# russellgeum/Digging-into-Self-Supervised-Monocular-Depth-Estimation

Hardware: AMD Instinct MI355X
Metric: images/sec training, KITTI 192x640 batch 12/GPU (higher is better)
Workload: dtype f32; 1 GPU; configs[1]: kitti_eigen_zhou-shaped 192x640, batch 12/GPU, ResNet18 depth + separate ResNet18 pose, frame_ids [0,-1,1], 4 scales, automask, Adam, fp32; global_batch=12, parallelism=dp1

## Files before the change

### digging-into-self-supervised-monocular-depth-estimation_amd/csrc/norm_nhwc.hip

```cpp
#include "nhwc_common.hpp"

namespace mdx {
namespace nhwc {

constexpr int STATS_FWD_BLOCKS = 256;
constexpr int STATS_BWD_BLOCKS_F32 = 256, STATS_BWD_BLOCKS_BF16 = 384;
constexpr int STATS_MAX_BLOCKS = 384;
constexpr int APPLY_MAX_BLOCKS = 4096;
constexpr int STATS_ITERS = 8, APPLY_ITERS = 4;
static inline int stats_bwd_blocks(int dtype) { return dtype == MDX_F32 ? STATS_BWD_BLOCKS_F32 : STATS_BWD_BLOCKS_BF16; }

template <typename T>
__global__ __launch_bounds__(NB) void bn_nhwc_fwd_stats_kernel(const T *__restrict__ x, int M, int C, int CVB, int PL, int RB,
                                                               float *__restrict__ part)
{
    constexpr int N = VecN<T>::N;
    __shared__ float lds[2 * NB * N];
    const Pos p = position<N>(M, C, CVB, PL, RB);
    float a[N], q[N];
#pragma unroll
    for (int j = 0; j < N; ++j) a[j] = q[j] = 0.f;
    if (p.active) {
        const T *px = x + (size_t)p.g * M * C + (size_t)p.cv * N;
        auto acc = [&](const Vec<T, N> &v) {
#pragma unroll
            for (int j = 0; j < N; ++j) {
                const float f = to_float(v.v[j]);
                a[j] += f;
                q[j] = __builtin_fmaf(f, f, q[j]);
            }
        };
        int r = p.r0 + p.pl;
        for (; r + 3 * PL < p.r1; r += 4 * PL) {
            const Vec<T, N> v0 = load_vec<T, N>(px + (size_t)r * C), v1 = load_vec<T, N>(px + (size_t)(r + PL) * C);
            const Vec<T, N> v2 = load_vec<T, N>(px + (size_t)(r + 2 * PL) * C), v3 = load_vec<T, N>(px + (size_t)(r + 3 * PL) * C);
            acc(v0); acc(v1); acc(v2); acc(v3);
        }
        for (; r < p.r1; r += PL) acc(load_vec<T, N>(px + (size_t)r * C));
    }
    block_partials<N>(a, q, lds, CVB, PL, C, part + ((size_t)p.g * gridDim.x + blockIdx.x) * 2 * C);
}

constexpr int FC = 16, FS = 64, FU = STATS_MAX_BLOCKS / FS;
__device__ __forceinline__ void channel_totals(const float *__restrict__ part_g, int nblk, int C, int c, double (*lds)[FS / 4][FC],
                                               double &ta, double &tq)
{
    const int cl = threadIdx.x % FC, sl = threadIdx.x / FC;
    float va[FU], vq[FU];
#pragma unroll
    for (int i = 0; i < FU; ++i) {
        const int b = sl + i * FS;
        const bool ok = c < C && b < nblk;
        va[i] = ok ? part_g[(size_t)b * 2 * C + c] : 0.f;
        vq[i] = ok ? part_g[(size_t)b * 2 * C + C + c] : 0.f;
    }
    double a = 0.0, q = 0.0;
#pragma unroll
    for (int i = 0; i < FU; ++i) {
        a += (double)va[i];
        q += (double)vq[i];
    }
    a += __shfl_down(a, 32, 64);
    q += __shfl_down(q, 32, 64);
    a += __shfl_down(a, 16, 64);
    q += __shfl_down(q, 16, 64);
    if ((threadIdx.x & 63) < FC) {
        lds[0][threadIdx.x >> 6][cl] = a;
        lds[1][threadIdx.x >> 6][cl] = q;
    }
    __syncthreads();
    ta = tq = 0.0;
    if (threadIdx.x < FC)
#pragma unroll
        for (int s = 0; s < FS / 4; ++s) {
            ta += lds[0][s][cl];
            tq += lds[1][s][cl];
        }
    __syncthreads();
}

__global__ __launch_bounds__(FC *FS) void bn_nhwc_fwd_finalize_kernel(const float *__restrict__ part, int nblk, int C, int G, double M,
                                                                       float eps, float momentum, float *__restrict__ save_mean,
                                                                       float *__restrict__ save_invstd, float *__restrict__ run_mean,
                                                                       float *__restrict__ run_var)
{
    __shared__ double lds[2][FS / 4][FC];
    const int c = blockIdx.x * FC + threadIdx.x % FC;
    const bool writer = threadIdx.x < FC && c < C;
    float rm = 0.f, rv = 0.f;
    if (writer && run_mean) { rm = run_mean[c]; rv = run_var[c]; }
    for (int g = 0; g < G; ++g) {
        double a, q;
        channel_totals(part + (size_t)g * nblk * 2 * C, nblk, C, c, lds, a, q);
        if (writer) {
            const double m = a / M;
            double var = q / M - m * m;
            var = var > 0.0 ? var : 0.0;
            const float mean = (float)m;
            save_mean[(size_t)g * C + c] = mean;
            save_invstd[(size_t)g * C + c] = (float)(1.0 / sqrt(var + (double)eps));
            const double unbiased = M > 1.0 ? var * (M / (M - 1.0)) : var;
            rm = (1.0f - momentum) * rm + momentum * mean;
            rv = (1.0f - momentum) * rv + momentum * (float)unbiased;
        }
    }
    if (writer && run_mean) { run_mean[c] = rm; run_var[c] = rv; }
}

__global__ __launch_bounds__(FC *FS) void bn_nhwc_bwd_finalize_kernel(const float *__restrict__ part, int nblk, int C, int G, double M,
                                                                       float *__restrict__ totals, float *__restrict__ dgamma,
                                                                       float *__restrict__ dbeta)
{
    __shared__ double lds[2][FS / 4][FC];
    const int c = blockIdx.x * FC + threadIdx.x % FC;
    const bool writer = threadIdx.x < FC && c < C;
    float sa = 0.f, sq = 0.f;
    for (int g = 0; g < G; ++g) {
        double a, q;
        channel_totals(part + (size_t)g * nblk * 2 * C, nblk, C, c, lds, a, q);
        if (writer) {
            totals[((size_t)g * 2 + 0) * C + c] = (float)((double)(float)a / M);
            totals[((size_t)g * 2 + 1) * C + c] = (float)((double)(float)q / M);
            sa += (float)a;
            sq += (float)q;
        }
    }
    if (writer) { dbeta[c] = sa; dgamma[c] = sq; }
}

template <typename T>
__global__ __launch_bounds__(NB) void bn_nhwc_fwd_apply_kernel(const T *__restrict__ x, const T *__restrict__ res,
                                                               const float *__restrict__ gamma, const float *__restrict__ beta,
                                                               const float *__restrict__ save_mean,
                                                               const float *__restrict__ save_invstd, int M, int C, int CVB, int PL,
                                                               int RB, int relu, T *__restrict__ y)
{
    constexpr int N = VecN<T>::N;
    const Pos p = position<N>(M, C, CVB, PL, RB);
    if (!p.active) return;
    float scale[N], shift[N];
#pragma unroll
    for (int j = 0; j < N; ++j) {
        const int c = p.cv * N + j;
        scale[j] = gamma[c] * save_invstd[(size_t)p.g * C + c];
        shift[j] = beta[c] - save_mean[(size_t)p.g * C + c] * scale[j];
    }
    const size_t base = (size_t)p.g * M * C + (size_t)p.cv * N;
    const T *px = x + base;
    const T *pr = res ? res + base : nullptr;
    T *py = y + base;
    auto apply = [&](const Vec<T, N> &v, const Vec<T, N> &rv, size_t off) {
        Vec<T, N> w;
#pragma unroll
        for (int j = 0; j < N; ++j) {
            float f = __builtin_fmaf(to_float(v.v[j]), scale[j], shift[j]);
            if (pr) f += to_float(rv.v[j]);
            w.v[j] = from_float<T>((relu && f < 0.f) ? 0.f : f);
        }
        store_vec<T, N>(py + off, w);
    };
    int r = p.r0 + p.pl;
    for (; r + 3 * PL < p.r1; r += 4 * PL) {
        const size_t o0 = (size_t)r * C, o1 = (size_t)(r + PL) * C, o2 = (size_t)(r + 2 * PL) * C, o3 = (size_t)(r + 3 * PL) * C;
        const Vec<T, N> v0 = load_vec<T, N>(px + o0), v1 = load_vec<T, N>(px + o1), v2 = load_vec<T, N>(px + o2), v3 = load_vec<T, N>(px + o3);
        Vec<T, N> r0 = {}, r1 = {}, r2 = {}, r3 = {};
        if (pr) { r0 = load_vec<T, N>(pr + o0); r1 = load_vec<T, N>(pr + o1); r2 = load_vec<T, N>(pr + o2); r3 = load_vec<T, N>(pr + o3); }
        apply(v0, r0, o0); apply(v1, r1, o1); apply(v2, r2, o2); apply(v3, r3, o3);
    }
    for (; r < p.r1; r += PL) {
        const size_t o = (size_t)r * C;
        Vec<T, N> rv = {};
        if (pr) rv = load_vec<T, N>(pr + o);
        apply(load_vec<T, N>(px + o), rv, o);
    }
}

template <typename T, bool MASKX>
__global__ __launch_bounds__(NB) void bn_nhwc_bwd_stats_kernel(const T *__restrict__ dy, const T *__restrict__ dy2,
                                                               const T *__restrict__ y, const T *__restrict__ x,
                                                               const float *__restrict__ gamma, const float *__restrict__ beta,
                                                               const float *__restrict__ save_mean,
                                                               const float *__restrict__ save_invstd, int M, int C, int CVB, int PL,
                                                               int RB, int relu, float *__restrict__ part)
{
    constexpr int N = VecN<T>::N;
    __shared__ float lds[2 * NB * N];
    const Pos p = position<N>(M, C, CVB, PL, RB);
    float a[N], q[N];
#pragma unroll
    for (int j = 0; j < N; ++j) a[j] = q[j] = 0.f;
    if (p.active) {
        float mean[N], invstd[N], scale[N], shift[N];
#pragma unroll
        for (int j = 0; j < N; ++j) {
            mean[j] = save_mean[(size_t)p.g * C + p.cv * N + j];
            invstd[j] = save_invstd[(size_t)p.g * C + p.cv * N + j];
            scale[j] = shift[j] = 0.f;
            if (MASKX) {
                scale[j] = gamma[p.cv * N + j] * invstd[j];
                shift[j] = beta[p.cv * N + j] - mean[j] * scale[j];
            }
        }
        const size_t base = (size_t)p.g * M * C + (size_t)p.cv * N;
        const T *pd = dy + base, *pd2 = dy2 ? dy2 + base : nullptr, *py = MASKX ? nullptr : y + base, *px = x + base;
        auto acc = [&](const Vec<T, N> &vd, const Vec<T, N> &vd2, const Vec<T, N> &vy, const Vec<T, N> &vx) {
#pragma unroll
            for (int j = 0; j < N; ++j) {
                float d = to_float(vd.v[j]);
                if (pd2) d += to_float(vd2.v[j]);
                const float yv = !MASKX ? to_float(vy.v[j]) : to_float(from_float<T>(__builtin_fmaf(to_float(vx.v[j]), scale[j], shift[j])));
                const float dz = (relu && !(yv > 0.f)) ? 0.f : d;
                a[j] += dz;
                q[j] = __builtin_fmaf(dz, (to_float(vx.v[j]) - mean[j]) * invstd[j], q[j]);
            }
        };
        int r = p.r0 + p.pl;
        for (; r + PL < p.r1; r += 2 * PL) {
            const size_t o0 = (size_t)r * C, o1 = (size_t)(r + PL) * C;
            const Vec<T, N> d0 = load_vec<T, N>(pd + o0), d1 = load_vec<T, N>(pd + o1);
            Vec<T, N> y0 = {}, y1 = {};
            if (!MASKX) { y0 = load_vec<T, N>(py + o0); y1 = load_vec<T, N>(py + o1); }
            const Vec<T, N> x0 = load_vec<T, N>(px + o0), x1 = load_vec<T, N>(px + o1);
            Vec<T, N> e0 = {}, e1 = {};
            if (pd2) { e0 = load_vec<T, N>(pd2 + o0); e1 = load_vec<T, N>(pd2 + o1); }
            acc(d0, e0, y0, x0);
            acc(d1, e1, y1, x1);
        }
        for (; r < p.r1; r += PL) {
            const size_t o = (size_t)r * C;
            Vec<T, N> e = {}, yv = {};
            if (pd2) e = load_vec<T, N>(pd2 + o);
            if (!MASKX) yv = load_vec<T, N>(py + o);
            acc(load_vec<T, N>(pd + o), e, yv, load_vec<T, N>(px + o));
        }
    }
    block_partials<N>(a, q, lds, CVB, PL, C, part + ((size_t)p.g * gridDim.x + blockIdx.x) * 2 * C);
}

template <typename T, bool MASKX>
__global__ __launch_bounds__(NB) void bn_nhwc_bwd_apply_kernel(const T *__restrict__ dy, const T *__restrict__ dy2,
                                                               const T *__restrict__ y, const T *__restrict__ x,
                                                               const float *__restrict__ gamma, const float *__restrict__ beta,
                                                               const float *__restrict__ save_mean,
                                                               const float *__restrict__ save_invstd,
                                                               const float *__restrict__ totals, int M, int C, int CVB, int PL,
                                                               int RB, int relu, T *__restrict__ dx, T *__restrict__ dres)
{
    constexpr int N = VecN<T>::N;
    const Pos p = position<N>(M, C, CVB, PL, RB);
    if (!p.active) return;
    float mean[N], invstd[N], k0[N], mdz[N], mdzx[N], shift[N];
#pragma unroll
    for (int j = 0; j < N; ++j) {
        const int c = p.cv * N + j;
        mean[j] = save_mean[(size_t)p.g * C + c];
        invstd[j] = save_invstd[(size_t)p.g * C + c];
        k0[j] = gamma[c] * invstd[j];
        shift[j] = MASKX ? beta[c] - mean[j] * k0[j] : 0.f;
        mdz[j] = totals[((size_t)p.g * 2 + 0) * C + c];
        mdzx[j] = totals[((size_t)p.g * 2 + 1) * C + c];
    }
    const size_t base = (size_t)p.g * M * C + (size_t)p.cv * N;
    const T *pd = dy + base, *pd2 = dy2 ? dy2 + base : nullptr, *py = MASKX ? nullptr : y + base, *px = x + base;
    T *ox = dx + base;
    T *orr = dres ? dres + base : nullptr;
    auto apply = [&](const Vec<T, N> &vd, const Vec<T, N> &vd2, const Vec<T, N> &vy, const Vec<T, N> &vx, size_t off) {
        Vec<T, N> wx, wr;
#pragma unroll
        for (int j = 0; j < N; ++j) {
            float d = to_float(vd.v[j]);
            if (pd2) d += to_float(vd2.v[j]);
            const float yv = !MASKX ? to_float(vy.v[j]) : to_float(from_float<T>(__builtin_fmaf(to_float(vx.v[j]), k0[j], shift[j])));
            const float dz = (relu && !(yv > 0.f)) ? 0.f : d;
            const float xh = (to_float(vx.v[j]) - mean[j]) * invstd[j];
            wx.v[j] = from_float<T>(k0[j] * (dz - mdz[j] - xh * mdzx[j]));
            wr.v[j] = from_float<T>(dz);
        }
        store_vec<T, N>(ox + off, wx);
        if (orr) store_vec<T, N>(orr + off, wr);
    };
    int r = p.r0 + p.pl;
    for (; r + PL < p.r1; r += 2 * PL) {
        const size_t o0 = (size_t)r * C, o1 = (size_t)(r + PL) * C;
        const Vec<T, N> d0 = load_vec<T, N>(pd + o0), d1 = load_vec<T, N>(pd + o1);
        Vec<T, N> y0 = {}, y1 = {};
        if (!MASKX) { y0 = load_vec<T, N>(py + o0); y1 = load_vec<T, N>(py + o1); }
        const Vec<T, N> x0 = load_vec<T, N>(px + o0), x1 = load_vec<T, N>(px + o1);
        Vec<T, N> e0 = {}, e1 = {};
        if (pd2) { e0 = load_vec<T, N>(pd2 + o0); e1 = load_vec<T, N>(pd2 + o1); }
        apply(d0, e0, y0, x0, o0);
        apply(d1, e1, y1, x1, o1);
    }
    for (; r < p.r1; r += PL) {
        const size_t o = (size_t)r * C;
        Vec<T, N> e = {}, yv = {};
        if (pd2) e = load_vec<T, N>(pd2 + o);
        if (!MASKX) yv = load_vec<T, N>(py + o);
        apply(load_vec<T, N>(pd + o), e, yv, load_vec<T, N>(px + o), o);
    }
}

}
}

using namespace mdx;
using namespace mdx::nhwc;

MDX_EXPORT size_t mdx_bn_nhwc_workspace_bytes(int B, int C, int H, int W, int groups, int dtype)
{
    if (B <= 0 || C <= 0 || H <= 0 || W <= 0 || groups <= 0 || !dtype_ok(dtype)) return 0;
    const Rows g = make_rows((long long)B * H * W, C, vec_elems(dtype), STATS_MAX_BLOCKS, STATS_ITERS);
    return ((size_t)groups * g.nblk * 2 * C + (size_t)groups * 2 * C) * sizeof(float);
}

static int nhwc_args_ok(int B, int C, int H, int W, int groups, int dtype)
{
    if (groups <= 0 || groups > 65535) return MDX_ERR_BAD_SHAPE;
    return nhwc_map_ok(B, C, H, W, dtype);
}

MDX_EXPORT int mdx_bn_act_nhwc_fwd(const void *x, const void *res, const float *gamma, const float *beta, float *run_mean,
                                   float *run_var, void *y, float *save_mean, float *save_invstd, int B, int C, int H, int W,
                                   int groups, float eps, float momentum, int relu, int dtype, void *workspace,
                                   size_t workspace_bytes, void *stream)
{
    if (!x || !gamma || !beta || !y || !save_mean || !save_invstd || !workspace) return MDX_ERR_NULL_POINTER;
    if ((run_mean == nullptr) != (run_var == nullptr)) return MDX_ERR_NULL_POINTER;
    const int bad = nhwc_args_ok(B, C, H, W, groups, dtype);
    if (bad) return bad;
    if (!aligned(x, 16) || !aligned(y, 16) || (res && !aligned(res, 16))) return MDX_ERR_MISALIGNED;
    if (workspace_bytes < mdx_bn_nhwc_workspace_bytes(B, C, H, W, groups, dtype)) return MDX_ERR_WORKSPACE;
    const int M = B * H * W, N = vec_elems(dtype);
    const Rows gs = make_rows(M, C, N, STATS_FWD_BLOCKS, STATS_ITERS), ga = make_rows(M, C, N, APPLY_MAX_BLOCKS, APPLY_ITERS);
    float *part = (float *)workspace;
    hipStream_t st = (hipStream_t)stream;
    const dim3 grid_s(gs.nblk, gs.t.ny, groups), grid_a(ga.nblk, ga.t.ny, groups), block(NB);
    dispatch_dtype(dtype, [&](auto t) {
        using T = typename decltype(t)::type;
        hipLaunchKernelGGL((bn_nhwc_fwd_stats_kernel<T>), grid_s, block, 0, st, (const T *)x, M, C, gs.t.CVB, gs.t.PL, gs.RB, part);
    });
    hipLaunchKernelGGL(bn_nhwc_fwd_finalize_kernel, dim3((C + FC - 1) / FC), dim3(FC * FS), 0, st, part, gs.nblk, C, groups, (double)M,
                       eps, momentum, save_mean, save_invstd, run_mean, run_var);
    dispatch_dtype(dtype, [&](auto t) {
        using T = typename decltype(t)::type;
        hipLaunchKernelGGL((bn_nhwc_fwd_apply_kernel<T>), grid_a, block, 0, st, (const T *)x, (const T *)res, gamma, beta, save_mean,
                           save_invstd, M, C, ga.t.CVB, ga.t.PL, ga.RB, relu, (T *)y);
    });
    return check_launch();
}

MDX_EXPORT int mdx_bn_act_nhwc_bwd(const void *dy, const void *dy2, const void *y, const void *x, const float *gamma,
                                   const float *beta, const float *save_mean, const float *save_invstd, void *dx, void *dres, float *dgamma,
                                   float *dbeta, int B, int C, int H, int W, int groups, int relu, int dtype, void *workspace,
                                   size_t workspace_bytes, void *stream)
{
    if (!dy || !x || !gamma || !save_mean || !save_invstd || !dx || !dgamma || !dbeta || !workspace)
        return MDX_ERR_NULL_POINTER;
    if (!y && (!relu || !beta || dres)) return MDX_ERR_NULL_POINTER;
    const int bad = nhwc_args_ok(B, C, H, W, groups, dtype);
    if (bad) return bad;
    if (!aligned(dy, 16) || (y && !aligned(y, 16)) || !aligned(x, 16) || !aligned(dx, 16) || (dy2 && !aligned(dy2, 16)) ||
        (dres && !aligned(dres, 16)))
        return MDX_ERR_MISALIGNED;
    if (workspace_bytes < mdx_bn_nhwc_workspace_bytes(B, C, H, W, groups, dtype)) return MDX_ERR_WORKSPACE;
    const int M = B * H * W, N = vec_elems(dtype);
    const Rows gs = make_rows(M, C, N, stats_bwd_blocks(dtype), STATS_ITERS), ga = make_rows(M, C, N, APPLY_MAX_BLOCKS, APPLY_ITERS);
    float *part = (float *)workspace;
    float *totals = part + (size_t)groups * gs.nblk * 2 * C;
    hipStream_t st = (hipStream_t)stream;
    const dim3 grid_s(gs.nblk, gs.t.ny, groups), grid_a(ga.nblk, ga.t.ny, groups), block(NB);
    const bool maskx = !y;
    dispatch_dtype_flag(dtype, maskx, [&](auto t, auto mx) {
        using T = typename decltype(t)::type;
        hipLaunchKernelGGL((bn_nhwc_bwd_stats_kernel<T, decltype(mx)::value>), grid_s, block, 0, st, (const T *)dy, (const T *)dy2,
                           (const T *)y, (const T *)x, gamma, beta, save_mean, save_invstd, M, C, gs.t.CVB, gs.t.PL, gs.RB, relu, part);
    });
    hipLaunchKernelGGL(bn_nhwc_bwd_finalize_kernel, dim3((C + FC - 1) / FC), dim3(FC * FS), 0, st, part, gs.nblk, C, groups, (double)M, totals,
                       dgamma, dbeta);
    dispatch_dtype_flag(dtype, maskx, [&](auto t, auto mx) {
        using T = typename decltype(t)::type;
        hipLaunchKernelGGL((bn_nhwc_bwd_apply_kernel<T, decltype(mx)::value>), grid_a, block, 0, st, (const T *)dy, (const T *)dy2,
                           (const T *)y, (const T *)x, gamma, beta, save_mean, save_invstd, totals, M, C, ga.t.CVB, ga.t.PL, ga.RB, relu,
                           (T *)dx, (T *)dres);
    });
    return check_launch();
}
```

### digging-into-self-supervised-monocular-depth-estimation_amd/csrc/pose_head_nhwc.hip

```cpp
#include "nhwc_common.hpp"

namespace mdx {
namespace nhwc {

constexpr int BA_BLOCKS = 256, BA_ITERS = 4;

template <typename T>
__global__ __launch_bounds__(NB) void bias_act_nhwc_fwd_kernel(const T *__restrict__ x, const float *__restrict__ bias, int M, int C,
                                                               int CVB, int PL, int RB, int relu, T *__restrict__ y)
{
    constexpr int N = VecN<T>::N;
    const Pos p = position<N>(M, C, CVB, PL, RB);
    if (!p.active) return;
    float b[N];
#pragma unroll
    for (int j = 0; j < N; ++j) b[j] = bias[p.cv * N + j];
    const T *px = x + (size_t)p.cv * N;
    T *py = y + (size_t)p.cv * N;
    for (int r = p.r0 + p.pl; r < p.r1; r += PL) {
        const Vec<T, N> v = load_vec<T, N>(px + (size_t)r * C);
        Vec<T, N> w;
#pragma unroll
        for (int j = 0; j < N; ++j) {
            const float f = to_float(v.v[j]) + b[j];
            w.v[j] = from_float<T>((relu && f < 0.f) ? 0.f : f);
        }
        store_vec<T, N>(py + (size_t)r * C, w);
    }
}

template <typename T>
__global__ __launch_bounds__(NB) void bias_act_nhwc_bwd_kernel(const T *__restrict__ dy, const T *__restrict__ y, int M, int C, int CVB,
                                                               int PL, int RB, int relu, T *__restrict__ dx, float *__restrict__ part)
{
    constexpr int N = VecN<T>::N;
    __shared__ float lds[NB * N];
    const Pos p = position<N>(M, C, CVB, PL, RB);
    float a[N];
#pragma unroll
    for (int j = 0; j < N; ++j) a[j] = 0.f;
    if (p.active) {
        const T *__restrict__ pd = dy + (size_t)p.cv * N, *__restrict__ py = y + (size_t)p.cv * N;
        T *__restrict__ ox = dx + (size_t)p.cv * N;
        auto one = [&](const Vec<T, N> &d, const Vec<T, N> &v, size_t off) {
            Vec<T, N> w;
#pragma unroll
            for (int j = 0; j < N; ++j) {
                const float dz = (relu && !(to_float(v.v[j]) > 0.f)) ? 0.f : to_float(d.v[j]);
                a[j] += dz;
                w.v[j] = from_float<T>(dz);
            }
            store_vec<T, N>(ox + off, w);
        };
        int r = p.r0 + p.pl;
        for (; r + 3 * PL < p.r1; r += 4 * PL) {
            const size_t o0 = (size_t)r * C, o1 = (size_t)(r + PL) * C, o2 = (size_t)(r + 2 * PL) * C, o3 = (size_t)(r + 3 * PL) * C;
            const Vec<T, N> d0 = load_vec<T, N>(pd + o0), d1 = load_vec<T, N>(pd + o1), d2 = load_vec<T, N>(pd + o2), d3 = load_vec<T, N>(pd + o3);
            const Vec<T, N> v0 = load_vec<T, N>(py + o0), v1 = load_vec<T, N>(py + o1), v2 = load_vec<T, N>(py + o2), v3 = load_vec<T, N>(py + o3);
            one(d0, v0, o0); one(d1, v1, o1); one(d2, v2, o2); one(d3, v3, o3);
        }
        for (; r < p.r1; r += PL) one(load_vec<T, N>(pd + (size_t)r * C), load_vec<T, N>(py + (size_t)r * C), (size_t)r * C);
    }
#pragma unroll
    for (int j = 0; j < N; ++j) lds[threadIdx.x * N + j] = a[j];
    __syncthreads();
    const int width = CVB * N;
    for (int e = threadIdx.x; e < width; e += NB) {
        const int c = blockIdx.y * width + e;
        if (c >= C) break;
        float s = 0.f;
        for (int l = 0; l < PL; ++l) s += lds[l * width + e];
        part[(size_t)blockIdx.x * C + c] = s;
    }
}

constexpr int PF_C = 16, PF_S = 64;
__global__ __launch_bounds__(PF_C *PF_S) void colsum_scale_kernel(const float *__restrict__ part, int n, int C, float scale,
                                                                  float *__restrict__ out)
{
    __shared__ float lds[PF_S / 4][PF_C];
    const int cl = threadIdx.x % PF_C, sl = threadIdx.x / PF_C, c = blockIdx.x * PF_C + cl;
    float s = 0.f;
    for (int i = sl; i < n; i += PF_S) s += (c < C) ? part[(size_t)i * C + c] : 0.f;
    s += __shfl_down(s, 32, 64);
    s += __shfl_down(s, 16, 64);
    if ((threadIdx.x & 63) < PF_C) lds[threadIdx.x >> 6][cl] = s;
    __syncthreads();
    if (threadIdx.x < PF_C && c < C) {
        float tot = 0.f;
#pragma unroll
        for (int k = 0; k < PF_S / 4; ++k) tot += lds[k][cl];
        out[c] = tot * scale;
    }
}

template <typename T>
__global__ __launch_bounds__(NB) void mean_bias_nhwc_fwd_kernel(const T *__restrict__ x, const float *__restrict__ bias, int M, int HW,
                                                                int C, float inv_hw, float scale, float *__restrict__ out)
{
    const int e = blockIdx.x * NB + threadIdx.x;
    if (e >= M * C) return;
    const int m = e / C, c = e - m * C;
    const T *px = x + (size_t)m * HW * C + c;
    float s0 = 0.f, s1 = 0.f, s2 = 0.f, s3 = 0.f;
    int p = 0;
    for (; p + 3 < HW; p += 4) {
        s0 += to_float(px[(size_t)p * C]); s1 += to_float(px[(size_t)(p + 1) * C]);
        s2 += to_float(px[(size_t)(p + 2) * C]); s3 += to_float(px[(size_t)(p + 3) * C]);
    }
    for (; p < HW; ++p) s0 += to_float(px[(size_t)p * C]);
    const float mean = ((s0 + s1) + (s2 + s3)) * inv_hw;
    out[e] = scale * (mean + (bias ? bias[c] : 0.f));
}

template <typename T>
__global__ __launch_bounds__(NB) void mean_bias_nhwc_bwd_kernel(const float *__restrict__ g, int M, int HW, int C, float inv_hw, float scale,
                                                                T *__restrict__ dx, float *__restrict__ dbias)
{
    const int e = blockIdx.x * NB + threadIdx.x;
    if (e >= M * C) return;
    const int m = e / C, c = e - m * C;
    const T v = from_float<T>((g[e] * scale) * inv_hw);
    T *px = dx + (size_t)m * HW * C + c;
    for (int p = 0; p < HW; ++p) px[(size_t)p * C] = v;
    if (m == 0 && dbias) {
        float s = 0.f;
        for (int i = 0; i < M; ++i) s += g[(size_t)i * C + c];
        dbias[c] = s * scale;
    }
}

static int ph_args_ok(long long M, int C, int dtype, bool vectors)
{
    if (!dtype_ok(dtype)) return MDX_ERR_BAD_SHAPE;
    if (M <= 0 || C <= 0 || M >= (1ll << 31) || M * C >= (1ll << 31)) return MDX_ERR_BAD_SHAPE;
    if (vectors && C % vec_elems(dtype)) return MDX_ERR_BAD_SHAPE;
    return MDX_OK;
}

}
}

using namespace mdx;
using namespace mdx::nhwc;

MDX_EXPORT size_t mdx_bias_act_nhwc_workspace_bytes(int B, int C, int H, int W, int dtype)
{
    const long long M = (long long)B * H * W;
    if (ph_args_ok(M, C, dtype, true)) return 0;
    return (size_t)make_rows(M, C, vec_elems(dtype), BA_BLOCKS, BA_ITERS).nblk * C * sizeof(float);
}

MDX_EXPORT int mdx_bias_act_nhwc_fwd(const void *x, const float *bias, void *y, int B, int C, int H, int W, int relu, int dtype,
                                     void *stream)
{
    if (!x || !bias || !y) return MDX_ERR_NULL_POINTER;
    const long long M = (long long)B * H * W;
    const int bad = ph_args_ok(M, C, dtype, true);
    if (bad) return bad;
    if (!aligned(x, 16) || !aligned(y, 16)) return MDX_ERR_MISALIGNED;
    const Rows g = make_rows(M, C, vec_elems(dtype), 4096, BA_ITERS);
    const dim3 grid(g.nblk, g.t.ny), block(NB);
    dispatch_dtype(dtype, [&](auto t) {
        using T = typename decltype(t)::type;
        hipLaunchKernelGGL((bias_act_nhwc_fwd_kernel<T>), grid, block, 0, (hipStream_t)stream, (const T *)x, bias, (int)M, C, g.t.CVB,
                           g.t.PL, g.RB, relu, (T *)y);
    });
    return check_launch();
}

MDX_EXPORT int mdx_bias_act_nhwc_bwd(const void *dy, const void *y, void *dx, float *dbias, int B, int C, int H, int W, int relu,
                                     int dtype, void *workspace, size_t workspace_bytes, void *stream)
{
    if (!dy || !y || !dx || !dbias || !workspace) return MDX_ERR_NULL_POINTER;
    const long long M = (long long)B * H * W;
    const int bad = ph_args_ok(M, C, dtype, true);
    if (bad) return bad;
    if (!aligned(dy, 16) || !aligned(y, 16) || !aligned(dx, 16)) return MDX_ERR_MISALIGNED;
    if (workspace_bytes < mdx_bias_act_nhwc_workspace_bytes(B, C, H, W, dtype)) return MDX_ERR_WORKSPACE;
    const Rows g = make_rows(M, C, vec_elems(dtype), BA_BLOCKS, BA_ITERS);
    const dim3 grid(g.nblk, g.t.ny), block(NB);
    float *part = (float *)workspace;
    hipStream_t st = (hipStream_t)stream;
    dispatch_dtype(dtype, [&](auto t) {
        using T = typename decltype(t)::type;
        hipLaunchKernelGGL((bias_act_nhwc_bwd_kernel<T>), grid, block, 0, st, (const T *)dy, (const T *)y, (int)M, C, g.t.CVB, g.t.PL,
                           g.RB, relu, (T *)dx, part);
    });
    hipLaunchKernelGGL(colsum_scale_kernel, dim3((C + PF_C - 1) / PF_C), dim3(PF_C * PF_S), 0, st, part, g.nblk, C, 1.0f, dbias);
    return check_launch();
}

MDX_EXPORT int mdx_mean_bias_nhwc_fwd(const void *x, const float *bias, float *out, int B, int C, int H, int W, float scale, int dtype,
                                      void *stream)
{
    if (!x || !out) return MDX_ERR_NULL_POINTER;
    const long long HW = (long long)H * W;
    const int bad = ph_args_ok((long long)B * HW, C, dtype, false);
    if (bad) return bad;
    const int n = B * C;
    const float inv = 1.0f / (float)HW;
    dispatch_dtype(dtype, [&](auto t) {
        using T = typename decltype(t)::type;
        hipLaunchKernelGGL((mean_bias_nhwc_fwd_kernel<T>), dim3((n + NB - 1) / NB), dim3(NB), 0, (hipStream_t)stream, (const T *)x, bias,
                           B, (int)HW, C, inv, scale, out);
    });
    return check_launch();
}

MDX_EXPORT int mdx_mean_bias_nhwc_bwd(const float *gout, void *dx, float *dbias, int B, int C, int H, int W, float scale, int dtype,
                                      void *stream)
{
    if (!gout || !dx) return MDX_ERR_NULL_POINTER;
    const long long HW = (long long)H * W;
    const int bad = ph_args_ok((long long)B * HW, C, dtype, false);
    if (bad) return bad;
    const int n = B * C;
    const float inv = 1.0f / (float)HW;
    dispatch_dtype(dtype, [&](auto t) {
        using T = typename decltype(t)::type;
        hipLaunchKernelGGL((mean_bias_nhwc_bwd_kernel<T>), dim3((n + NB - 1) / NB), dim3(NB), 0, (hipStream_t)stream, gout, B, (int)HW,
                           C, inv, scale, (T *)dx, dbias);
    });
    return check_launch();
}

namespace mdx {
namespace nhwc {

struct InputSrc { const float *p[4]; };

template <typename T>
__global__ __launch_bounds__(NB) void encoder_input_nhwc_kernel(InputSrc src, int groups, int n, int HW, float mean, float inv_std,
                                                                T *__restrict__ out)
{
    const int pix = blockIdx.x * NB + threadIdx.x, img = blockIdx.y;
    if (pix >= HW) return;
    const int k = img >= n ? 1 : 0, b = img - k * n;
    const int C = 3 * groups;
    float v[6];
#pragma unroll
    for (int g = 0; g < 2; ++g) {
        if (g >= groups) break;
        const float *__restrict__ s = (k == 0 ? (g == 0 ? src.p[0] : src.p[1]) : (g == 0 ? src.p[2] : src.p[3])) + (size_t)b * 3 * HW + pix;
#pragma unroll
        for (int c = 0; c < 3; ++c) v[3 * g + c] = (s[(size_t)c * HW] - mean) * inv_std;
    }
    T *o = out + ((size_t)img * HW + pix) * C;
#pragma unroll
    for (int c = 0; c < 6; ++c)
        if (c < C) o[c] = from_float<T>(v[c]);
}

}
}

MDX_EXPORT int mdx_encoder_input_nhwc(const float *const *src, int blocks, int groups, int n, int H, int W, float mean, float inv_std,
                                      void *out, int dtype, void *stream)
{
    if (!src || !out) return MDX_ERR_NULL_POINTER;
    if (blocks < 1 || blocks > 2 || groups < 1 || groups > 2 || n <= 0 || H <= 0 || W <= 0) return MDX_ERR_BAD_SHAPE;
    if (!dtype_ok(dtype)) return MDX_ERR_BAD_SHAPE;
    const long long total = (long long)blocks * n * H * W;
    if (total * 6 >= (1ll << 40)) return MDX_ERR_BAD_SHAPE;
    InputSrc s = {{nullptr, nullptr, nullptr, nullptr}};
    for (int k = 0; k < blocks; ++k)
        for (int g = 0; g < groups; ++g) {
            if (!src[k * groups + g]) return MDX_ERR_NULL_POINTER;
            s.p[2 * k + g] = src[k * groups + g];
        }
    if ((long long)H * W >= (1ll << 31) || blocks * n > 65535) return MDX_ERR_BAD_SHAPE;
    const dim3 grid((unsigned)(((long long)H * W + NB - 1) / NB), (unsigned)(blocks * n));
    dispatch_dtype(dtype, [&](auto t) {
        using T = typename decltype(t)::type;
        hipLaunchKernelGGL((encoder_input_nhwc_kernel<T>), grid, dim3(NB), 0, (hipStream_t)stream, s, groups, n, H * W, mean, inv_std,
                           (T *)out);
    });
    return check_launch();
}
```

### digging-into-self-supervised-monocular-depth-estimation_amd/csrc/thinconv_nhwc.hip

```cpp
#include "nhwc_common.hpp"

namespace mdx {
namespace nhwc {

typedef float v4f __attribute__((ext_vector_type(4)));
constexpr int TW_WAVES = 4;

template <int CIN>
__global__ __launch_bounds__(64 * TW_WAVES) void thin_wgrad16_kernel(const float *__restrict__ x, const float *__restrict__ gy, int B, int h,
                                                                      int w, int quads_per_wave, float *__restrict__ part)
{
    constexpr int CH = CIN / 16, NT = 9 * CH;
    __shared__ float lds[TW_WAVES][256];
    const int lane = threadIdx.x & 63, wave = threadIdx.x >> 6;
    const int Hp = h + 2, Wp = w + 2, wq = w / 4;
    const long long nquads = (long long)B * h * wq;
    const long long q0 = ((long long)blockIdx.x * TW_WAVES + wave) * quads_per_wave;
    const long long q1 = q0 + quads_per_wave < nquads ? q0 + quads_per_wave : nquads;
    v4f acc[NT];
#pragma unroll
    for (int t = 0; t < NT; ++t) acc[t] = (v4f){0.f, 0.f, 0.f, 0.f};
    const int k = lane >> 4, j = lane & 15;
    if (q0 < q1) {
        int qx = (int)(q0 % wq);
        const long long row0 = q0 / wq;
        int i = (int)(row0 % h);
        const int b0 = (int)(row0 / h);
        const float *pg = gy + (size_t)q0 * 64 + lane;
        const float *px = x + (((size_t)b0 * Hp + i) * Wp + (size_t)qx * 4 + k) * CIN + j;
        auto load_b = [&](const float *xb, float (&bv)[NT]) {
#pragma unroll
            for (int ty = 0; ty < 3; ++ty)
#pragma unroll
                for (int tx = 0; tx < 3; ++tx)
#pragma unroll
                    for (int c = 0; c < CH; ++c) bv[(ty * 3 + tx) * CH + c] = xb[((size_t)ty * Wp + tx) * CIN + c * 16];
        };
        auto advance = [&]() {
            pg += 64;
            px += 4 * CIN;
            if (++qx == wq) {
                qx = 0;
                px += 2 * CIN;
                if (++i == h) { i = 0; px += (size_t)2 * Wp * CIN; }
            }
        };
        float a0 = *pg, b0v[NT];
        load_b(px, b0v);
        for (long long q = q0; q < q1; ++q) {
            float a1 = 0.f, b1v[NT];
            advance();
            if (q + 1 < q1) {
                a1 = *pg;
                load_b(px, b1v);
            } else {
#pragma unroll
                for (int t = 0; t < NT; ++t) b1v[t] = 0.f;
            }
#pragma unroll
            for (int t = 0; t < NT; ++t) acc[t] = __builtin_amdgcn_mfma_f32_16x16x4f32(a0, b0v[t], acc[t], 0, 0, 0);
            a0 = a1;
#pragma unroll
            for (int t = 0; t < NT; ++t) b0v[t] = b1v[t];
        }
    }
    float *dst = part + (size_t)blockIdx.x * NT * 256;
#pragma unroll
    for (int t = 0; t < NT; ++t) {
#pragma unroll
        for (int v = 0; v < 4; ++v) lds[wave][(4 * k + v) * 16 + j] = acc[t][v];
        __syncthreads();
        {
            const int r = threadIdx.x;
            float s = lds[0][r];
#pragma unroll
            for (int u = 1; u < TW_WAVES; ++u) s += lds[u][r];
            dst[t * 256 + r] = s;
        }
        __syncthreads();
    }
}

constexpr int TF_S = 64;
__global__ __launch_bounds__(16 * TF_S) void thin_wgrad16_finish_kernel(const float *__restrict__ part, int nblk, int CIN, long wso, long wsc,
                                                                        long wsy, long wsx, float *__restrict__ gw)
{
    __shared__ float lds[TF_S / 4][16];
    const int n = 9 * CIN * 16;
    const int cl = threadIdx.x % 16, sl = threadIdx.x / 16, e = blockIdx.x * 16 + cl;
    float s = 0.f;
    for (int i = sl; i < nblk; i += TF_S) s += (e < n) ? part[(size_t)i * n + e] : 0.f;
    s += __shfl_down(s, 32, 64);
    s += __shfl_down(s, 16, 64);
    if ((threadIdx.x & 63) < 16) lds[threadIdx.x >> 6][cl] = s;
    __syncthreads();
    if (threadIdx.x < 16 && e < n) {
        float tot = 0.f;
#pragma unroll
        for (int u = 0; u < TF_S / 4; ++u) tot += lds[u][cl];
        const int CH = CIN / 16;
        const int t = e >> 8, r = e & 255, co = r >> 4, cj = r & 15;
        const int tap = t / CH, ci = (t % CH) * 16 + cj;
        gw[co * wso + ci * wsc + (tap / 3) * wsy + (tap % 3) * wsx] = tot;
    }
}

struct ThinGeom { int blocks, quads_per_wave; };
static inline ThinGeom thin_geom(int B, int h, int w)
{
    const long long nquads = (long long)B * h * (w / 4);
    ThinGeom g;
    long long waves = 6144;
    if (waves * 48 > nquads) waves = (nquads + 47) / 48;
    if (waves < 1) waves = 1;
    g.quads_per_wave = (int)((nquads + waves - 1) / waves);
    g.blocks = (int)((nquads + (long long)g.quads_per_wave * TW_WAVES - 1) / ((long long)g.quads_per_wave * TW_WAVES));
    return g;
}

}
}

using namespace mdx;
using namespace mdx::nhwc;

static int thin_args_ok(int B, int Cin, int Cout, int h, int w)
{
    if (B <= 0 || h <= 0 || w <= 0 || w % 4 || Cout != 16 || (Cin != 16 && Cin != 32)) return MDX_ERR_BAD_SHAPE;
    if ((long long)B * (h + 2) * (w + 2) * Cin >= (1ll << 40)) return MDX_ERR_BAD_SHAPE;
    return MDX_OK;
}

MDX_EXPORT size_t mdx_thin_conv3x3_wgrad_workspace_bytes(int B, int Cin, int Cout, int h, int w)
{
    if (thin_args_ok(B, Cin, Cout, h, w)) return 0;
    return (size_t)thin_geom(B, h, w).blocks * 9 * Cin * 16 * sizeof(float);
}

MDX_EXPORT int mdx_thin_conv3x3_wgrad(const float *x, const float *gy, float *gweight, int64_t s_o, int64_t s_c, int64_t s_y, int64_t s_x,
                                      int B, int Cin, int Cout, int h, int w, void *workspace, size_t workspace_bytes, void *stream)
{
    if (!x || !gy || !gweight || !workspace) return MDX_ERR_NULL_POINTER;
    const int bad = thin_args_ok(B, Cin, Cout, h, w);
    if (bad) return bad;
    if (workspace_bytes < mdx_thin_conv3x3_wgrad_workspace_bytes(B, Cin, Cout, h, w)) return MDX_ERR_WORKSPACE;
    const ThinGeom g = thin_geom(B, h, w);
    float *part = (float *)workspace;
    hipStream_t st = (hipStream_t)stream;
    if (Cin == 16)
        hipLaunchKernelGGL((thin_wgrad16_kernel<16>), dim3(g.blocks), dim3(64 * TW_WAVES), 0, st, x, gy, B, h, w, g.quads_per_wave, part);
    else
        hipLaunchKernelGGL((thin_wgrad16_kernel<32>), dim3(g.blocks), dim3(64 * TW_WAVES), 0, st, x, gy, B, h, w, g.quads_per_wave, part);
    const int n = 9 * Cin * 16;
    hipLaunchKernelGGL(thin_wgrad16_finish_kernel, dim3((n + 15) / 16), dim3(16 * TF_S), 0, st, part, g.blocks, Cin, (long)s_o, (long)s_c,
                       (long)s_y, (long)s_x, gweight);
    return check_launch();
}
```

Baseline: 823.1 images/s.

## Batch partial loads in BN finalize and pose-head kernels, stage encoder input stores

BN finalize kernels now issue the partial-sum loads for the next group (or both groups when G==2) before reducing the current one, with clamped unconditional loads so memory latency overlaps. The mean-bias forward splits each channel reduction over four lanes with 32-deep batched loads and shuffle-combines the lanes. The mean-bias backward and the thin-conv wgrad finish kernel batch their strided loads the same way. The encoder input kernel stages NHWC outputs in LDS and writes them with aligned vector stores instead of scalar 3/6-channel stores. Together these target latency-bound small kernels at the cost of more registers, added LDS use and a barrier.

```diff
diff --git a/digging-into-self-supervised-monocular-depth-estimation_amd/csrc/norm_nhwc.hip b/digging-into-self-supervised-monocular-depth-estimation_amd/csrc/norm_nhwc.hip
--- a/digging-into-self-supervised-monocular-depth-estimation_amd/csrc/norm_nhwc.hip
+++ b/digging-into-self-supervised-monocular-depth-estimation_amd/csrc/norm_nhwc.hip
@@ -42,18 +42,26 @@
 }
 
 constexpr int FC = 16, FS = 64, FU = STATS_MAX_BLOCKS / FS;
-__device__ __forceinline__ void channel_totals(const float *__restrict__ part_g, int nblk, int C, int c, double (*lds)[FS / 4][FC],
-                                               double &ta, double &tq)
-{
-    const int cl = threadIdx.x % FC, sl = threadIdx.x / FC;
-    float va[FU], vq[FU];
+struct Partials { float a[FU], q[FU]; };
+__device__ __forceinline__ Partials load_partials(const float *__restrict__ part_g, int nblk, int C, int c)
+{
+    const int sl = threadIdx.x / FC, cc = min(c, C - 1);
+    Partials v;
 #pragma unroll
     for (int i = 0; i < FU; ++i) {
         const int b = sl + i * FS;
         const bool ok = c < C && b < nblk;
-        va[i] = ok ? part_g[(size_t)b * 2 * C + c] : 0.f;
-        vq[i] = ok ? part_g[(size_t)b * 2 * C + C + c] : 0.f;
-    }
+        const float *p = part_g + (size_t)min(b, nblk - 1) * 2 * C + cc;
+        const float a = p[0], q = p[C];
+        v.a[i] = ok ? a : 0.f;
+        v.q[i] = ok ? q : 0.f;
+    }
+    return v;
+}
+__device__ __forceinline__ void channel_totals(const Partials &v, double (*lds)[FS / 4][FC], double &ta, double &tq)
+{
+    const int cl = threadIdx.x % FC;
+    const float (&va)[FU] = v.a, (&vq)[FU] = v.q;
     double a = 0.0, q = 0.0;
 #pragma unroll
     for (int i = 0; i < FU; ++i) {
@@ -79,6 +87,31 @@
     __syncthreads();
 }
 
+template <typename F>
+__device__ __forceinline__ void for_group_totals(const float *__restrict__ part, int nblk, int C, int G, int c, double (*lds)[FS / 4][FC],
+                                                 F &&f)
+{
+    const size_t stride = (size_t)nblk * 2 * C;
+    double a, q;
+    if (G == 2) {
+        const Partials p0 = load_partials(part, nblk, C, c), p1 = load_partials(part + stride, nblk, C, c);
+        __builtin_amdgcn_sched_barrier(0);
+        channel_totals(p0, lds, a, q);
+        f(0, a, q);
+        channel_totals(p1, lds, a, q);
+        f(1, a, q);
+        return;
+    }
+    Partials cur = load_partials(part, nblk, C, c);
+    for (int g = 0; g < G; ++g) {
+        Partials nxt = cur;
+        if (g + 1 < G) nxt = load_partials(part + (size_t)(g + 1) * stride, nblk, C, c);
+        channel_totals(cur, lds, a, q);
+        f(g, a, q);
+        cur = nxt;
+    }
+}
+
 __global__ __launch_bounds__(FC *FS) void bn_nhwc_fwd_finalize_kernel(const float *__restrict__ part, int nblk, int C, int G, double M,
                                                                        float eps, float momentum, float *__restrict__ save_mean,
                                                                        float *__restrict__ save_invstd, float *__restrict__ run_mean,
@@ -89,9 +122,7 @@
     const bool writer = threadIdx.x < FC && c < C;
     float rm = 0.f, rv = 0.f;
     if (writer && run_mean) { rm = run_mean[c]; rv = run_var[c]; }
-    for (int g = 0; g < G; ++g) {
-        double a, q;
-        channel_totals(part + (size_t)g * nblk * 2 * C, nblk, C, c, lds, a, q);
+    for_group_totals(part, nblk, C, G, c, lds, [&](int g, double a, double q) {
         if (writer) {
             const double m = a / M;
             double var = q / M - m * m;
@@ -103,7 +134,7 @@
             rm = (1.0f - momentum) * rm + momentum * mean;
             rv = (1.0f - momentum) * rv + momentum * (float)unbiased;
         }
-    }
+    });
     if (writer && run_mean) { run_mean[c] = rm; run_var[c] = rv; }
 }
 
@@ -115,16 +146,14 @@
     const int c = blockIdx.x * FC + threadIdx.x % FC;
     const bool writer = threadIdx.x < FC && c < C;
     float sa = 0.f, sq = 0.f;
-    for (int g = 0; g < G; ++g) {
-        double a, q;
-        channel_totals(part + (size_t)g * nblk * 2 * C, nblk, C, c, lds, a, q);
+    for_group_totals(part, nblk, C, G, c, lds, [&](int g, double a, double q) {
         if (writer) {
             totals[((size_t)g * 2 + 0) * C + c] = (float)((double)(float)a / M);
             totals[((size_t)g * 2 + 1) * C + c] = (float)((double)(float)q / M);
             sa += (float)a;
             sq += (float)q;
         }
-    }
+    });
     if (writer) { dbeta[c] = sa; dgamma[c] = sq; }
 }
 
diff --git a/digging-into-self-supervised-monocular-depth-estimation_amd/csrc/pose_head_nhwc.hip b/digging-into-self-supervised-monocular-depth-estimation_amd/csrc/pose_head_nhwc.hip
--- a/digging-into-self-supervised-monocular-depth-estimation_amd/csrc/pose_head_nhwc.hip
+++ b/digging-into-self-supervised-monocular-depth-estimation_amd/csrc/pose_head_nhwc.hip
@@ -94,40 +94,60 @@
     }
 }
 
+constexpr int MB_U = 32;
 template <typename T>
 __global__ __launch_bounds__(NB) void mean_bias_nhwc_fwd_kernel(const T *__restrict__ x, const float *__restrict__ bias, int M, int HW,
                                                                 int C, float inv_hw, float scale, float *__restrict__ out)
+{
+    const long long t = (long long)blockIdx.x * NB + threadIdx.x;
+    const int j = (int)(t & 3);
+    if ((t >> 2) >= (long long)M * C) return;
+    const int e = (int)(t >> 2), m = e / C, c = e - m * C;
+    const T *px = x + (size_t)m * HW * C + c;
+    const int nq = HW >> 2;
+    float tail[3];
+#pragma unroll
+    for (int i = 0; i < 3; ++i) tail[i] = (j == 0 && 4 * nq + i < HW) ? to_float(px[(size_t)(4 * nq + i) * C]) : 0.f;
+    float s = 0.f;
+    for (int q0 = 0; q0 < nq; q0 += MB_U) {
+        float v[MB_U];
+#pragma unroll
+        for (int i = 0; i < MB_U; ++i) v[i] = q0 + i < nq ? to_float(px[(size_t)(4 * (q0 + i) + j) * C]) : 0.f;
+#pragma unroll
+        for (int i = 0; i < MB_U; ++i)
+            if (q0 + i < nq) s += v[i];
+    }
+#pragma unroll
+    for (int i = 0; i < 3; ++i)
+        if (j == 0 && 4 * nq + i < HW) s += tail[i];
+    s += __shfl_xor(s, 1, 64);
+    s += __shfl_xor(s, 2, 64);
+    if (j == 0) out[e] = scale * (s * inv_hw + (bias ? bias[c] : 0.f));
+}
+
+template <typename T>
+__global__ __launch_bounds__(NB) void mean_bias_nhwc_bwd_kernel(const float *__restrict__ g, int M, int HW, int C, float inv_hw, float scale,
+                                                                T *__restrict__ dx, float *__restrict__ dbias)
 {
     const int e = blockIdx.x * NB + threadIdx.x;
     if (e >= M * C) return;
     const int m = e / C, c = e - m * C;
-    const T *px = x + (size_t)m * HW * C + c;
-    float s0 = 0.f, s1 = 0.f, s2 = 0.f, s3 = 0.f;
-    int p = 0;
-    for (; p + 3 < HW; p += 4) {
-        s0 += to_float(px[(size_t)p * C]); s1 += to_float(px[(size_t)(p + 1) * C]);
-        s2 += to_float(px[(size_t)(p + 2) * C]); s3 += to_float(px[(size_t)(p + 3) * C]);
-    }
-    for (; p < HW; ++p) s0 += to_float(px[(size_t)p * C]);
-    const float mean = ((s0 + s1) + (s2 + s3)) * inv_hw;
-    out[e] = scale * (mean + (bias ? bias[c] : 0.f));
-}
-
-template <typename T>
-__global__ __launch_bounds__(NB) void mean_bias_nhwc_bwd_kernel(const float *__restrict__ g, int M, int HW, int C, float inv_hw, float scale,
-                                                                T *__restrict__ dx, float *__restrict__ dbias)
-{
-    const int e = blockIdx.x * NB + threadIdx.x;
-    if (e >= M * C) return;
-    const int m = e / C, c = e - m * C;
-    const T v = from_float<T>((g[e] * scale) * inv_hw);
+    const float ge = g[e];
+    if (m == 0 && dbias) {
+        float s = 0.f;
+        for (int i0 = 0; i0 < M; i0 += MB_U) {
+            float v[MB_U];
+#pragma unroll
+            for (int i = 0; i < MB_U; ++i) v[i] = i0 + i < M ? g[(size_t)(i0 + i) * C + c] : 0.f;
+#pragma unroll
+            for (int i = 0; i < MB_U; ++i)
+                if (i0 + i < M) s += v[i];
+        }
+        dbias[c] = s * scale;
+    }
+    const T v = from_float<T>((ge * scale) * inv_hw);
     T *px = dx + (size_t)m * HW * C + c;
     for (int p = 0; p < HW; ++p) px[(size_t)p * C] = v;
-    if (m == 0 && dbias) {
-        float s = 0.f;
-        for (int i = 0; i < M; ++i) s += g[(size_t)i * C + c];
-        dbias[c] = s * scale;
-    }
 }
 
 static int ph_args_ok(long long M, int C, int dtype, bool vectors)
@@ -198,11 +218,11 @@
     const long long HW = (long long)H * W;
     const int bad = ph_args_ok((long long)B * HW, C, dtype, false);
     if (bad) return bad;
-    const int n = B * C;
+    const long long n = 4ll * B * C;
     const float inv = 1.0f / (float)HW;
     dispatch_dtype(dtype, [&](auto t) {
         using T = typename decltype(t)::type;
-        hipLaunchKernelGGL((mean_bias_nhwc_fwd_kernel<T>), dim3((n + NB - 1) / NB), dim3(NB), 0, (hipStream_t)stream, (const T *)x, bias,
+        hipLaunchKernelGGL((mean_bias_nhwc_fwd_kernel<T>), dim3((unsigned)((n + NB - 1) / NB)), dim3(NB), 0, (hipStream_t)stream, (const T *)x, bias,
                            B, (int)HW, C, inv, scale, out);
     });
     return check_launch();
@@ -234,22 +254,37 @@
 __global__ __launch_bounds__(NB) void encoder_input_nhwc_kernel(InputSrc src, int groups, int n, int HW, float mean, float inv_std,
                                                                 T *__restrict__ out)
 {
-    const int pix = blockIdx.x * NB + threadIdx.x, img = blockIdx.y;
-    if (pix >= HW) return;
+    constexpr int N = VecN<T>::N;
+    __shared__ Vec<T, N> stage[(NB * 6 + N) / N + 1];
+    T *lds = reinterpret_cast<T *>(stage);
+    const int pix0 = blockIdx.x * NB, pix = pix0 + threadIdx.x, img = blockIdx.y;
     const int k = img >= n ? 1 : 0, b = img - k * n;
     const int C = 3 * groups;
-    float v[6];
-#pragma unroll
-    for (int g = 0; g < 2; ++g) {
-        if (g >= groups) break;
-        const float *__restrict__ s = (k == 0 ? (g == 0 ? src.p[0] : src.p[1]) : (g == 0 ? src.p[2] : src.p[3])) + (size_t)b * 3 * HW + pix;
-#pragma unroll
-        for (int c = 0; c < 3; ++c) v[3 * g + c] = (s[(size_t)c * HW] - mean) * inv_std;
-    }
-    T *o = out + ((size_t)img * HW + pix) * C;
-#pragma unroll
-    for (int c = 0; c < 6; ++c)
-        if (c < C) o[c] = from_float<T>(v[c]);
+    const int np = min(NB, HW - pix0), ne = np * C;
+    T *o = out + ((size_t)img * HW + pix0) * C;
+    const int sh = (int)(((uintptr_t)o / sizeof(T)) % N);
+    if (pix < HW) {
+        float v[6];
+#pragma unroll
+        for (int g = 0; g < 2; ++g) {
+            if (g >= groups) break;
+            const float *__restrict__ s = (k == 0 ? (g == 0 ? src.p[0] : src.p[1]) : (g == 0 ? src.p[2] : src.p[3])) + (size_t)b * 3 * HW + pix;
+#pragma unroll
+            for (int c = 0; c < 3; ++c) v[3 * g + c] = (s[(size_t)c * HW] - mean) * inv_std;
+        }
+#pragma unroll
+        for (int c = 0; c < 6; ++c)
+            if (c < C) lds[sh + threadIdx.x * C + c] = from_float<T>(v[c]);
+    }
+    __syncthreads();
+    const int head = min(ne, (N - sh) % N);
+    const int nv = (ne - head) / N;
+    for (int i = threadIdx.x; i < nv; i += NB) store_vec<T, N>(o + head + i * N, stage[(sh + head) / N + i]);
+    const int rest = ne - nv * N;
+    if ((int)threadIdx.x < rest) {
+        const int e = (int)threadIdx.x < head ? (int)threadIdx.x : nv * N + (int)threadIdx.x;
+        o[e] = lds[sh + e];
+    }
 }
 
 }
diff --git a/digging-into-self-supervised-monocular-depth-estimation_amd/csrc/thinconv_nhwc.hip b/digging-into-self-supervised-monocular-depth-estimation_amd/csrc/thinconv_nhwc.hip
--- a/digging-into-self-supervised-monocular-depth-estimation_amd/csrc/thinconv_nhwc.hip
+++ b/digging-into-self-supervised-monocular-depth-estimation_amd/csrc/thinconv_nhwc.hip
@@ -81,7 +81,7 @@
     }
 }
 
-constexpr int TF_S = 64;
+constexpr int TF_S = 64, TF_U = 8;
 __global__ __launch_bounds__(16 * TF_S) void thin_wgrad16_finish_kernel(const float *__restrict__ part, int nblk, int CIN, long wso, long wsc,
                                                                         long wsy, long wsx, float *__restrict__ gw)
 {
@@ -89,7 +89,14 @@
     const int n = 9 * CIN * 16;
     const int cl = threadIdx.x % 16, sl = threadIdx.x / 16, e = blockIdx.x * 16 + cl;
     float s = 0.f;
-    for (int i = sl; i < nblk; i += TF_S) s += (e < n) ? part[(size_t)i * n + e] : 0.f;
+    const float *pe = part + min(e, n - 1);
+    for (int i0 = sl; i0 < nblk; i0 += TF_S * TF_U) {
+        float v[TF_U];
+#pragma unroll
+        for (int u = 0; u < TF_U; ++u) v[u] = pe[(size_t)min(i0 + u * TF_S, nblk - 1) * n];
+#pragma unroll
+        for (int u = 0; u < TF_U; ++u) s += (e < n && i0 + u * TF_S < nblk) ? v[u] : 0.f;
+    }
     s += __shfl_down(s, 32, 64);
     s += __shfl_down(s, 16, 64);
     if ((threadIdx.x & 63) < 16) lds[threadIdx.x >> 6][cl] = s;
```

New measurement: 824.0 images/s (median of 3 runs). About the same (+0.1%).
